# EPFL-VILAB/MultiMAE

Measured on NVIDIA H100. Metric: MultiMAE-B pretrain samples/sec @ bs=128/GPU, higher is better.
Workload: dtype bf16

## Files before the change

### include/multimae_b200.h

```cpp
#ifndef MULTIMAE_B200_H_
#define MULTIMAE_B200_H_

#include <stdint.h>

#ifdef __cplusplus
extern "C" {
#endif

#define MMAE_ABI_VERSION 15

int mmae_abi_version(void);
const char* mmae_last_error(void);
int64_t mmae_launch_count(void);

int mmae_profile_gemm(int enable);
int mmae_profile_gemm_read(double* flops, double* ms, int64_t* launches);
int64_t mmae_profile_gemm_dump(char* buf_host, int64_t capacity);

typedef struct mmae_gemm_epilogue {
  float alpha;
  int act;
  int accumulate;
  int reserved;
  const float* bias;
  const float* residual;
  const void* dgelu_z;
  void* preact_bf16;
  float* out_f32;
  void* out_bf16;
  int64_t ld_residual, ld_dgelu_z, ld_preact, ld_out_f32, ld_out_bf16;
} mmae_gemm_epilogue;

int mmae_gemm_set_variant(int variant);
int mmae_gemm_set_tma_store(int enable);
int mmae_set_pdl(int enable);
int mmae_set_sm_budget(int sms);
int mmae_set_wgrad_stream(int enable);

int mmae_gemm_bf16(const void* A, int64_t lda, int a_mn_major, const void* B, int64_t ldb, int b_mn_major,
                   int M, int N, int K, int split_k, const mmae_gemm_epilogue* ep, void* stream);

int mmae_cast_f32_to_bf16(const float* src, void* dst_bf16, int64_t n, void* stream);
int mmae_cast_colsum_f32(const float* src, int64_t ld_src, void* dst_bf16, int64_t ld_dst, float* colsum,
                         int M, int N, void* stream);
int mmae_colsum_bf16(const void* src_bf16, int64_t ld_src, float* colsum, int M, int N, void* stream);
int mmae_gelu_bf16(const void* z, void* io, int64_t n, int backward, void* stream);
int mmae_dgelu_colsum_bf16(const void* z, void* dz, int64_t ld, float* colsum, int M, int N, void* stream);
int mmae_set_fuse_gelu(int enable);
int mmae_add_bf16_f32(const float* x, const void* y_bf16, float* out, int64_t n, void* stream);
int mmae_transpose_bf16(const void* src, int64_t ld_src, void* dst, int64_t ld_dst, int M, int N, void* stream);

int mmae_layernorm_forward(const float* x, int64_t ldx, const float* gamma, const float* beta, void* y_bf16,
                           int64_t ldy, float* y_f32, int64_t ldyf, float* mean, float* rstd, int M, int D,
// ... 318 lines not shown
```

### multimae_b200/_lib.py

```python
import ctypes
import os

_HERE = os.path.dirname(os.path.abspath(__file__))
LIB_PATH = os.path.join(_HERE, "libmultimae_b200.so")

c_void_p = ctypes.c_void_p
c_int = ctypes.c_int
c_i64 = ctypes.c_int64
c_float = ctypes.c_float


class GemmEpilogue(ctypes.Structure):
    _fields_ = [
        ("alpha", c_float),
        ("act", c_int),
        ("accumulate", c_int),
        ("reserved", c_int),
        ("bias", c_void_p),
        ("residual", c_void_p),
        ("dgelu_z", c_void_p),
        ("preact_bf16", c_void_p),
        ("out_f32", c_void_p),
        ("out_bf16", c_void_p),
        ("ld_residual", c_i64),
        ("ld_dgelu_z", c_i64),
        ("ld_preact", c_i64),
        ("ld_out_f32", c_i64),
        ("ld_out_bf16", c_i64),
    ]


MAX_TASKS = 8
c_float_p = c_void_p
POS_MODES = {"bicubic": 0, "bilinear": 1}


class EmbedLayout(ctypes.Structure):
    _fields_ = [
        ("num_tasks", c_int),
        ("grid_h", c_int * MAX_TASKS), ("grid_w", c_int * MAX_TASKS),
        ("tok_offset", c_int * (MAX_TASKS + 1)),
        ("k_offset", c_int * (MAX_TASKS + 1)),
        ("patch", c_int * MAX_TASKS), ("channels", c_int * MAX_TASKS),
        ("is_semseg", c_int * MAX_TASKS), ("num_classes", c_int * MAX_TASKS),
    ]


class EmbedInputs(ctypes.Structure):
    _fields_ = [("data", c_void_p * MAX_TASKS), ("class_emb", c_void_p * MAX_TASKS)]


# ... 232 lines not shown
    "mmae_block_f32_saved_bytes": (c_i64, [c_int] * 5),
    "mmae_block_f32_workspace_bytes": (c_i64, [c_int] * 5),
    "mmae_block_f32_forward": (c_int, [c_void_p, c_void_p, c_int, c_int, c_int, c_int, c_int, c_float, c_void_p, c_void_p,
                                       ctypes.POINTER(BlockParams), c_void_p, c_void_p, c_void_p]),
    "mmae_block_f32_backward": (c_int, [c_void_p, c_void_p, c_void_p, c_int, c_int, c_int, c_int, c_int, c_void_p, c_void_p,
                                        ctypes.POINTER(BlockParams), ctypes.POINTER(BlockGrads), c_void_p, c_void_p,
                                        c_void_p]),
    "mmae_dechead_f32_saved_bytes": (c_i64, [ctypes.POINTER(DecoderIndex), c_int, c_int, c_int]),
    "mmae_dechead_f32_workspace_bytes": (c_i64, [ctypes.POINTER(DecoderIndex), c_int, c_int, c_int]),
    "mmae_dechead_f32_forward": (c_int, [c_void_p, c_int, ctypes.POINTER(DecoderIndex), c_int, c_int, c_float,
                                         ctypes.POINTER(DecHeadParams), c_void_p, c_void_p, c_void_p, c_void_p]),
    "mmae_dechead_f32_backward": (c_int, [c_void_p, c_int, ctypes.POINTER(DecoderIndex), c_int, c_int,
                                          ctypes.POINTER(DecHeadParams), ctypes.POINTER(DecHeadGrads), c_void_p, c_void_p,
                                          c_void_p, c_void_p, c_void_p]),
    "mmae_dectail_f32_workspace_bytes": (c_i64, [c_int] * 6),
    "mmae_dectail_f32_forward": (c_int, [c_void_p, c_int, c_int, c_int, c_int, c_int, c_int, c_void_p, c_void_p, c_void_p,
                                         c_void_p, c_void_p]),
    "mmae_dectail_f32_backward": (c_int, [c_void_p, c_void_p, c_int, c_int, c_int, c_int, c_int, c_int, c_void_p, c_void_p,
                                          c_void_p, c_void_p, c_void_p, c_void_p]),
    "mmae_standardize_depth_set_variant": (c_int, [c_int]),
    "mmae_standardize_depth": (c_int, [c_void_p, c_void_p, c_int, c_int, c_int, c_int, c_float, c_void_p, c_void_p]),
}

ABI_VERSION = 15


def lib():
    global _lib
    if _lib is not None:
        return _lib
    if not os.path.exists(LIB_PATH):
        raise MmaeError(
            "multimae_b200: %s is missing - build it with `python -m multimae_b200.build` "
            "(there is no CPU fallback)" % LIB_PATH)
    handle = ctypes.CDLL(LIB_PATH)
    for name, (res, args) in SIGNATURES.items():
        fn = getattr(handle, name)
        fn.restype = res
        fn.argtypes = args
    ver = handle.mmae_abi_version()
    if ver != ABI_VERSION:
        raise MmaeError("multimae_b200: ABI version mismatch (library %d, binding %d)" % (ver, ABI_VERSION))
    _lib = handle
    return _lib


def check(rc, what=""):
# ... 13 lines not shown
```

### multimae_b200/csrc/gemm_wgmma.cu

```cuda
#include <algorithm>
#include <cstdlib>

#include "common.cuh"
#include "../../include/multimae_b200.h"

namespace mmae {

void count_launch();
bool gemm_profile_begin(cudaStream_t st, double flops, int M, int N, int K, int flags);
void gemm_profile_end(cudaStream_t st);

namespace {

constexpr int BM = 128;
constexpr int BK = 64;
constexpr int WG_K = 16;
constexpr int GEMM_THREADS = 384;

struct GemmParams {
  int M, N, K;
  int num_kb;
  int kb_per_split;
  int tiles_n;
  int tiles_m;
  int splits;
  int tma_store;
  mmae_gemm_epilogue ep;
};

template <int BN>
struct GemmCfg {
  static constexpr int STAGES = BN == 256 ? 4 : (BN == 192 ? 4 : (BN == 128 ? 6 : 8));
  static constexpr int A_BYTES = BM * BK * 2;
  static constexpr int B_BYTES = BN * BK * 2;
  static constexpr int STAGE_BYTES = A_BYTES + B_BYTES;
  static constexpr int EPI_BOX_BYTES = 64 * 32 * 4;
  static constexpr int EPI_OFFSET = STAGES * STAGE_BYTES;
  static constexpr int BAR_OFFSET = EPI_OFFSET + 2 * 2 * EPI_BOX_BYTES;
  static constexpr int TOTAL = BAR_OFFSET + 256 + 1024;
  static_assert(TOTAL <= 232448, "GEMM exceeds the 227 KB shared-memory limit");
};

struct WorkItem {
  int m0, n0, split, kb_begin, nkb;
};

template <int BN, int CL>
__device__ __forceinline__ WorkItem decode_item(int item, const GemmParams& p, int rank) {
  WorkItem w;
  const int rest = item / p.tiles_n;
  w.n0 = (item - rest * p.tiles_n) * BN;
  w.split = rest / p.tiles_m;
  w.m0 = ((rest - w.split * p.tiles_m) * CL + rank) * BM;
  w.kb_begin = w.split * p.kb_per_split;
  w.nkb = min(p.kb_per_split, p.num_kb - w.kb_begin);
  return w;
}

__device__ __forceinline__ void red_add_v2(float* addr, float a, float b) {
  asm volatile("red.global.add.v2.f32 [%0], {%1, %2};" ::"l"(addr), "f"(a), "f"(b) : "memory");
}

__device__ __forceinline__ void epilogue_pair(float v0, float v1, int row, int n, const GemmParams& p, bool first_split,
                                              bool atomic_out) {
  const mmae_gemm_epilogue& ep = p.ep;
  v0 *= ep.alpha;
  v1 *= ep.alpha;
  if (ep.bias && first_split) {
    const float2 b = __ldg(reinterpret_cast<const float2*>(ep.bias + n));
    v0 += b.x;
    v1 += b.y;
  }
  if (ep.preact_bf16)
    *reinterpret_cast<uint32_t*>(reinterpret_cast<bf16*>(ep.preact_bf16) + int64_t(row) * ep.ld_preact + n) = pack_bf16x2(v0, v1);
  if (ep.act == 1) {
    v0 = gelu_erf(v0);
    v1 = gelu_erf(v1);
  }
  if (ep.dgelu_z) {
    const uint32_t z = __ldg(reinterpret_cast<const unsigned int*>(reinterpret_cast<const bf16*>(ep.dgelu_z) +
                                                                   int64_t(row) * ep.ld_dgelu_z + n));
    const float2 zf = unpack_bf16x2(z);
    v0 *= dgelu_erf(zf.x);
    v1 *= dgelu_erf(zf.y);
  }
  if (ep.residual && first_split) {
    const float2 r = __ldg(reinterpret_cast<const float2*>(ep.residual + int64_t(row) * ep.ld_residual + n));
    v0 += r.x;
    v1 += r.y;
  }
  if (ep.out_f32) {
    float* dst = ep.out_f32 + int64_t(row) * ep.ld_out_f32 + n;
    if (atomic_out) red_add_v2(dst, v0, v1);
    else *reinterpret_cast<float2*>(dst) = make_float2(v0, v1);
  }
  if (ep.out_bf16)
    *reinterpret_cast<uint32_t*>(reinterpret_cast<bf16*>(ep.out_bf16) + int64_t(row) * ep.ld_out_bf16 + n) = pack_bf16x2(v0, v1);
}

template <typename T>
__device__ __forceinline__ void stage_pair(uint8_t* box, int r, int c, float v0, float v1) {
  T* b = reinterpret_cast<T*>(box);
  if constexpr (sizeof(T) == 4) *reinterpret_cast<float2*>(b + r * 32 + c) = make_float2(v0, v1);
  else *reinterpret_cast<uint32_t*>(b + r * 32 + c) = pack_bf16x2(v0, v1);
}

template <int BN, int CL, bool A_MN, bool B_MN>
__global__ void __launch_bounds__(GEMM_THREADS, 1)
    gemm_bf16_kernel(const __grid_constant__ CUtensorMap tmA, const __grid_constant__ CUtensorMap tmB,
                     const __grid_constant__ CUtensorMap tmC, const GemmParams p) {
  pdl_launch_dependents();
  using C = GemmCfg<BN>;
  constexpr int STAGES = C::STAGES;
  constexpr int BH = BN / CL;
  static_assert(!B_MN || BH % 64 == 0, "MN-major B is loaded in 64-column chunks");

  extern __shared__ uint8_t smem_raw[];
  const uint32_t raw_addr = smem_u32(smem_raw);
  uint8_t* smem = smem_raw + ((1024u - (raw_addr & 1023u)) & 1023u);
  uint64_t* full_bar = reinterpret_cast<uint64_t*>(smem + C::BAR_OFFSET);
  uint64_t* empty_bar = full_bar + STAGES;

  const int wg = threadIdx.x >> 7;
  const int rank = CL > 1 ? int(cluster_ctarank()) : 0;
  const int num_items = p.tiles_n * p.tiles_m * p.splits;
  const int first_item = blockIdx.x / CL;
  const int item_stride = gridDim.x / CL;

  if (threadIdx.x == 0) {
    tma_prefetch_desc(&tmA);
    tma_prefetch_desc(&tmB);
    if (p.tma_store) tma_prefetch_desc(&tmC);
#pragma unroll
    for (int s = 0; s < STAGES; ++s) {
      mbar_init(&full_bar[s], 1);
      mbar_init(&empty_bar[s], 2 * CL);
    }
    fence_barrier_init();
  }
  __syncthreads();
  if constexpr (CL > 1) cluster_sync_all();
  pdl_wait();

  if (wg == 0) {
    setmaxnreg_dec<40>();
    if (threadIdx.x == 0) {
      uint32_t it = 0;
      for (int item = first_item; item < num_items; item += item_stride) {
        const WorkItem w = decode_item<BN, CL>(item, p, rank);
        for (int kb = 0; kb < w.nkb; ++kb, ++it) {
          const int s = it % STAGES;
          const uint32_t ph = (it / STAGES) & 1;
          mbar_wait(&empty_bar[s], ph ^ 1u);
          mbar_expect_tx(&full_bar[s], C::STAGE_BYTES);
          uint8_t* sA = smem + s * C::STAGE_BYTES;
          uint8_t* sB = sA + C::A_BYTES;
          const int k0 = (w.kb_begin + kb) * BK;
          if constexpr (!A_MN) {
            tma_load_2d(sA, &tmA, &full_bar[s], k0, w.m0);
          } else {
// ... 9 lines not shown
            }
          } else {
            if constexpr (!B_MN) {
              tma_load_2d_multicast(sB + rank * BH * 128, &tmB, &full_bar[s], k0, w.n0 + rank * BH, 0x3);
            } else {
#pragma unroll
              for (int c = 0; c < BH / 64; ++c)
                tma_load_2d_multicast(sB + (rank * (BH / 64) + c) * (64 * BK * 2), &tmB, &full_bar[s],
                                      w.n0 + rank * BH + c * 64, k0, 0x3);
            }
          }
        }
      }
    }
  } else {
    setmaxnreg_inc<232>();
    const int cw = wg - 1;
    const int t = threadIdx.x & 127;
    const int rl = (t >> 5) * 16 + ((t & 31) >> 2);
    uint8_t* epi = smem + C::EPI_OFFSET + cw * (2 * C::EPI_BOX_BYTES);
    const bool atomic_out = p.ep.accumulate != 0 || p.splits > 1;
    uint32_t it = 0;
    uint32_t boxes = 0;
    auto release = [&](int s) {
      if (t == 0) {
        if constexpr (CL == 1) mbar_arrive(&empty_bar[s]);
        else
          for (int r = 0; r < CL; ++r) mbar_arrive_cluster(mapa_u32(smem_u32(&empty_bar[s]), uint32_t(r)));
      }
    };
    float acc[BN / 2];

    for (int item = first_item; item < num_items; item += item_stride) {
      const WorkItem w = decode_item<BN, CL>(item, p, rank);
      for (int kb = 0; kb < w.nkb; ++kb, ++it) {
        const int s = it % STAGES;
        const uint32_t ph = (it / STAGES) & 1;
        mbar_wait(&full_bar[s], ph);
        const uint32_t a_addr = smem_u32(smem + s * C::STAGE_BYTES) + cw * (64 * BK * 2);
        const uint32_t b_addr = smem_u32(smem + s * C::STAGE_BYTES) + C::A_BYTES;
#pragma unroll
        for (int i = 0; i < BN / 2; ++i) reg_fence(acc[i]);
        wgmma_fence();
#pragma unroll
        for (int j = 0; j < BK / WG_K; ++j) {
          const uint32_t sd = (kb | j) != 0 ? 1u : 0u;
          const uint64_t da = A_MN ? gmma_desc_sw128(a_addr + j * (WG_K * 128), 64 * BK * 2, 1024)
                                   : gmma_desc_sw128(a_addr + j * (WG_K * 2), 16, 1024);
          const uint64_t db = B_MN ? gmma_desc_sw128(b_addr + j * (WG_K * 128), 64 * BK * 2, 1024)
                                   : gmma_desc_sw128(b_addr + j * (WG_K * 2), 16, 1024);
          if constexpr (BN == 256) wgmma_m64n256k16<A_MN ? 1 : 0, B_MN ? 1 : 0>(acc, da, db, sd);
          else if constexpr (BN == 192) wgmma_m64n192k16<A_MN ? 1 : 0, B_MN ? 1 : 0>(acc, da, db, sd);
          else if constexpr (BN == 128) wgmma_m64n128k16<A_MN ? 1 : 0, B_MN ? 1 : 0>(acc, da, db, sd);
          else wgmma_m64n64k16<A_MN ? 1 : 0, B_MN ? 1 : 0>(acc, da, db, sd);
        }
        wgmma_commit();
#pragma unroll
        for (int i = 0; i < BN / 2; ++i) reg_fence(acc[i]);
        wgmma_wait<1>();
        if (kb > 0) release((it - 1) % STAGES);
      }
      wgmma_wait<0>();
#pragma unroll
      for (int i = 0; i < BN / 2; ++i) reg_fence(acc[i]);
      release((it - 1) % STAGES);

      const int row_a = w.m0 + cw * 64 + rl;
      const int row_b = row_a + 8;
      const bool first_split = w.split == 0;
      if (p.tma_store) {
        const float* bias = first_split ? p.ep.bias : nullptr;
        const bool bf16_out = p.tma_store == 1;
#pragma unroll
        for (int b = 0; b < BN / 32; ++b) {
          if (w.n0 + b * 32 >= p.N) break;
          uint8_t* box = bf16_out ? epi + (boxes & 3) * (C::EPI_BOX_BYTES / 2) : epi + (boxes & 1) * C::EPI_BOX_BYTES;
          if (t == 0) {
            if (bf16_out) bulk_wait_read<3>();
            else bulk_wait_read<1>();
          }
          asm volatile("bar.sync %0, 128;" ::"r"(2 + cw) : "memory");
#pragma unroll
          for (int jj = 0; jj < 4; ++jj) {
            const int j = 4 * b + jj;
            const int c = jj * 8 + 2 * (t & 3);
            float v[4] = {acc[4 * j] * p.ep.alpha, acc[4 * j + 1] * p.ep.alpha, acc[4 * j + 2] * p.ep.alpha,
                          acc[4 * j + 3] * p.ep.alpha};
            if (bias && w.n0 + b * 32 + c < p.N) {
              const float2 bb = __ldg(reinterpret_cast<const float2*>(bias + w.n0 + b * 32 + c));
              v[0] += bb.x; v[1] += bb.y; v[2] += bb.x; v[3] += bb.y;
            }
            if (p.ep.act == 1) {
#pragma unroll
              for (int i = 0; i < 4; ++i) v[i] = gelu_erf(v[i]);
            }
            if (bf16_out) {
              stage_pair<bf16>(box, rl, c, v[0], v[1]);
              stage_pair<bf16>(box, rl + 8, c, v[2], v[3]);
            } else {
              stage_pair<float>(box, rl, c, v[0], v[1]);
              stage_pair<float>(box, rl + 8, c, v[2], v[3]);
            }
          }
          fence_proxy_async_smem();
          asm volatile("bar.sync %0, 128;" ::"r"(2 + cw) : "memory");
          if (t == 0) {
            if (p.tma_store == 3) tma_reduce_add_2d(&tmC, box, w.n0 + b * 32, w.m0 + cw * 64);
            else tma_store_2d(&tmC, box, w.n0 + b * 32, w.m0 + cw * 64);
            bulk_commit_group();
          }
          ++boxes;
        }
      } else {
#pragma unroll
        for (int j = 0; j < BN / 8; ++j) {
          if (w.n0 + j * 8 >= p.N) break;
          const int n = w.n0 + j * 8 + 2 * (t & 3);
          if (row_a < p.M) epilogue_pair(acc[4 * j], acc[4 * j + 1], row_a, n, p, first_split, atomic_out);
          if (row_b < p.M) epilogue_pair(acc[4 * j + 2], acc[4 * j + 3], row_b, n, p, first_split, atomic_out);
        }
      }
    }
    if (t == 0 && p.tma_store) bulk_wait_all();
  }
  if constexpr (CL > 1) cluster_sync_all();
}

template <int BN, int CL, bool A_MN, bool B_MN>
int launch_gemm(const CUtensorMap& tmA, const CUtensorMap& tmB, const CUtensorMap& tmC, const GemmParams& p,
                cudaStream_t stream) {
  using C = GemmCfg<BN>;
  auto kern = gemm_bf16_kernel<BN, CL, A_MN, B_MN>;
  cudaLaunchConfig_t cfg;
  memset(&cfg, 0, sizeof(cfg));
  cfg.blockDim = dim3(GEMM_THREADS);
  cfg.dynamicSmemBytes = C::TOTAL;
  cfg.stream = stream;
  cudaLaunchAttribute attr[2];
  attr[0].id = cudaLaunchAttributeClusterDimension;
  attr[0].val.clusterDim.x = CL;
  attr[0].val.clusterDim.y = 1;
  attr[0].val.clusterDim.z = 1;
  attr[1].id = cudaLaunchAttributeProgrammaticStreamSerialization;
  attr[1].val.programmaticStreamSerializationAllowed = 1;
  cfg.attrs = attr;
  cfg.numAttrs = 1;
  static int resident = 0;
  if (resident == 0) {
    MMAE_CUDA_OK(cudaFuncSetAttribute(kern, cudaFuncAttributeMaxDynamicSharedMemorySize, C::TOTAL));
    if constexpr (CL > 1) {
      cfg.gridDim = dim3(CL);
      MMAE_CUDA_OK(cudaOccupancyMaxActiveClusters(&resident, kern, &cfg));
    } else {
      int dev = 0, sms = 0;
      MMAE_CUDA_OK(cudaGetDevice(&dev));
      MMAE_CUDA_OK(cudaDeviceGetAttribute(&sms, cudaDevAttrMultiProcessorCount, dev));
      resident = sms;
    }
    MMAE_CHECK(resident > 0, MMAE_ERR_CUDA, "mmae_gemm_bf16: the GEMM kernel does not fit on an SM");
  }
  const int items = p.tiles_n * p.tiles_m * p.splits;
  const int slots = std::min(resident, std::max(1, sm_count() / CL));
  cfg.gridDim = dim3(std::min(items, slots) * CL);
  const bool prof = gemm_profile_begin(stream, 2.0 * p.M * p.N * p.K, p.M, p.N, p.K,
                                       (A_MN ? 1 : 0) | (B_MN ? 2 : 0) | (p.splits << 8));
  if constexpr (CL == 1) {
    cfg.attrs = attr + 1;
    cfg.numAttrs = pdl_enabled() ? 1 : 0;
  } else {
    cfg.numAttrs = pdl_enabled() ? 2 : 1;
  }
  MMAE_CUDA_OK(cudaLaunchKernelEx(&cfg, kern, tmA, tmB, tmC, p));
  if (prof) gemm_profile_end(stream);
  count_launch();
  MMAE_LAUNCH_OK();
  return MMAE_OK;
}

}
}

using namespace mmae;

static int g_gemm_variant = []() {
  const char* e = getenv("MMAE_GEMM_VARIANT");
  const int v = e ? atoi(e) : -1;
  return v >= -1 && v <= 6 ? v : -1;
}();
static int g_gemm_tma_store = []() {
  const char* e = getenv("MMAE_GEMM_TMA_STORE");
  return e ? (atoi(e) != 0) : 1;
}();

extern "C" int mmae_gemm_set_variant(int variant) {
  MMAE_CHECK(variant >= -1 && variant <= 6, MMAE_ERR_ARG, "mmae_gemm_set_variant: %d (-1 .. 6)", variant);
// ... 1 lines not shown
  return MMAE_OK;
}

extern "C" int mmae_gemm_set_tma_store(int enable) {
  g_gemm_tma_store = enable != 0;
  return MMAE_OK;
}

static int variant_bn(int v) { return v == 0 ? 64 : (v == 1 || v == 6) ? 128 : (v == 3 || v == 5) ? 192 : 256; }

constexpr int KB_PER_ITEM_FIXED = 4;
constexpr int MIN_KB_PER_SPLIT = 16;

extern "C" int mmae_gemm_bf16(const void* A, int64_t lda, int a_mn_major, const void* B, int64_t ldb,
                              int b_mn_major, int M, int N, int K, int split_k, const mmae_gemm_epilogue* ep,
                              void* stream) {
  MMAE_CHECK(A && B && ep, MMAE_ERR_ARG, "mmae_gemm_bf16: null operand");
  MMAE_CHECK(M > 0 && N > 0 && K > 0, MMAE_ERR_ARG, "mmae_gemm_bf16: bad shape M=%d N=%d K=%d", M, N, K);
  MMAE_CHECK(N % 8 == 0, MMAE_ERR_ARG, "mmae_gemm_bf16: N=%d must be a multiple of 8", N);
  MMAE_CHECK(lda % 8 == 0 && ldb % 8 == 0, MMAE_ERR_ARG, "mmae_gemm_bf16: lda/ldb must be multiples of 8");
  MMAE_CHECK((reinterpret_cast<uintptr_t>(A) & 15) == 0 && (reinterpret_cast<uintptr_t>(B) & 15) == 0,
             MMAE_ERR_ARG, "mmae_gemm_bf16: operands must be 16-byte aligned");
  MMAE_CHECK(ep->out_f32 || ep->out_bf16, MMAE_ERR_ARG, "mmae_gemm_bf16: no output");
  const int num_kb = ceil_div(K, BK);
  const int sms = sm_count();
  const int tm = ceil_div(M, BM);
  if (split_k <= 0 && !(ep->out_f32 && !ep->out_bf16 && !ep->preact_bf16 && !ep->dgelu_z && ep->act == 0)) split_k = 1;

  int variant = g_gemm_variant;
  {
    const int cand_var[2] = {1, 2};
    const int nvar = variant >= 0 ? 1 : 2;
    long best_cost = -1;
    int best_split = 1, best_var = variant >= 0 ? variant : 1;
    for (int i = 0; i < nvar; ++i) {
      const int v = variant >= 0 ? variant : cand_var[i];
      const int bn = variant_bn(v), cl = v >= 4 ? 2 : 1;
      if (variant < 0 && bn > 128 && N < bn) continue;
      const long tiles = long(ceil_div(tm, cl)) * ceil_div(N, bn);
      const int slots = std::max(1, sms / cl);
      const int s_lo = split_k > 0 ? split_k : 1;
      const int s_hi = split_k > 0 ? split_k : std::max(1, num_kb / MIN_KB_PER_SPLIT);
      for (int s = s_lo; s <= s_hi; ++s) {
        const int kbps = ceil_div(num_kb, std::min(s, num_kb));
        const long rounds = (tiles * ceil_div(num_kb, kbps) + slots - 1) / slots;
        const long cost = rounds * (bn + 40) * cl * (kbps + KB_PER_ITEM_FIXED);
// ... 30 lines not shown
  int rc;
  if (!a_mn_major) {
    rc = make_tmap_2d_bf16(&tmA, A, (uint64_t)M, (uint64_t)K, (uint64_t)lda, BK, BM);
  } else {
    MMAE_CHECK(M % 8 == 0, MMAE_ERR_ARG, "mmae_gemm_bf16: MN-major A needs M %% 8 == 0");
    rc = make_tmap_2d_bf16(&tmA, A, (uint64_t)K, (uint64_t)M, (uint64_t)lda, 64, BK);
  }
  if (rc) return rc;
  if (!b_mn_major) {
    rc = make_tmap_2d_bf16(&tmB, B, (uint64_t)N, (uint64_t)K, (uint64_t)ldb, BK, BNsel / CLsel);
  } else {
    rc = make_tmap_2d_bf16(&tmB, B, (uint64_t)K, (uint64_t)N, (uint64_t)ldb, 64, BK);
  }
  if (rc) return rc;

  GemmParams p;
  p.M = M; p.N = N; p.K = K;
  p.num_kb = num_kb;
  p.kb_per_split = kb_per_split;
  p.tiles_n = ceil_div(N, BNsel);
  p.tiles_m = ceil_div(tm, CLsel);
  p.splits = split_k;
  p.ep = *ep;
  p.tma_store = 0;
  CUtensorMap tmC = tmA;
  if (g_gemm_tma_store && !ep->preact_bf16 && !ep->dgelu_z && !ep->residual) {
    if (ep->out_bf16 && !ep->out_f32 && split_k == 1 && !ep->accumulate) {
      p.tma_store = 1;
      rc = make_tmap_2d_store(&tmC, ep->out_bf16, 2, (uint64_t)M, (uint64_t)N, (uint64_t)ep->ld_out_bf16);
      if (rc) return rc;
    } else if (ep->out_f32 && !ep->out_bf16 && ep->act == 0) {
      p.tma_store = (split_k > 1 || ep->accumulate) ? 3 : 2;
      rc = make_tmap_2d_store(&tmC, ep->out_f32, 4, (uint64_t)M, (uint64_t)N, (uint64_t)ep->ld_out_f32);
      if (rc) return rc;
    }
  }
  cudaStream_t st = reinterpret_cast<cudaStream_t>(stream);
#define MMAE_DISPATCH(BN_, CL_)                                                                      \
  do {                                                                                               \
    if (!a_mn_major && !b_mn_major) return launch_gemm<BN_, CL_, false, false>(tmA, tmB, tmC, p, st); \
    if (!a_mn_major && b_mn_major) return launch_gemm<BN_, CL_, false, true>(tmA, tmB, tmC, p, st);   \
    if (a_mn_major && !b_mn_major) return launch_gemm<BN_, CL_, true, false>(tmA, tmB, tmC, p, st);   \
    return launch_gemm<BN_, CL_, true, true>(tmA, tmB, tmC, p, st);                                  \
  } while (0)
  if (variant == 4) MMAE_DISPATCH(256, 2);
  if (variant == 6) MMAE_DISPATCH(128, 2);
  if (variant == 5) {
    if (!a_mn_major) return launch_gemm<192, 2, false, false>(tmA, tmB, tmC, p, st);
    return launch_gemm<192, 2, true, false>(tmA, tmB, tmC, p, st);
  }
  if (variant == 0) MMAE_DISPATCH(64, 1);
  if (variant == 3) MMAE_DISPATCH(192, 1);
  if (variant == 2) MMAE_DISPATCH(256, 1);
  MMAE_DISPATCH(128, 1);
#undef MMAE_DISPATCH
}
```

### multimae_b200/csrc/modules.cu

```cuda
#include <cstdlib>

#include "internal.h"

namespace mmae {
namespace {

struct Carver {
  uint8_t* base;
  size_t off = 0;
  explicit Carver(void* b) : base(reinterpret_cast<uint8_t*>(b)) {}
  template <typename T>
  T* take(size_t n) {
    off = align_up(off, 256);
    T* p = reinterpret_cast<T*>(base + off);
    off += n * sizeof(T);
    return p;
  }
};

}


int pick_split(int, int, int) { return 0; }

// ... 17 lines not shown
  ep.bias = b;
  ep.out_bf16 = y;
  ep.ld_out_bf16 = N;
  return mmae_gemm_bf16(x, K, 0, W, K, 0, M, N, K, 1, &ep, st);
}
int linear_f32(const bf16* x, const bf16* W, const float* b, const float* resid, float* y, int M, int N, int K,
               void* st) {
  mmae_gemm_epilogue ep = ep_zero();
  ep.bias = b;
  ep.residual = resid;
  ep.ld_residual = N;
  ep.out_f32 = y;
  ep.ld_out_f32 = N;
  return mmae_gemm_bf16(x, K, 0, W, K, 0, M, N, K, 1, &ep, st);
}
int g_fuse_gelu = []() {
  const char* e = getenv("MMAE_FUSE_GELU");
  return e ? atoi(e) : 0;
}();

int linear_gelu(const bf16* x, const bf16* W, const float* b, bf16* z, bf16* a, int M, int N, int K, void* st) {
  mmae_gemm_epilogue ep = ep_zero();
  ep.bias = b;
  if (g_fuse_gelu) {
    ep.act = 1;
    ep.preact_bf16 = z;
    ep.ld_preact = N;
    ep.out_bf16 = a;
    ep.ld_out_bf16 = N;
    return mmae_gemm_bf16(x, K, 0, W, K, 0, M, N, K, 1, &ep, st);
  }
  ep.out_bf16 = z;
  ep.ld_out_bf16 = N;
  int rc = mmae_gemm_bf16(x, K, 0, W, K, 0, M, N, K, 1, &ep, st);
  if (rc != MMAE_OK) return rc;
  return mmae_gelu_bf16(z, a, int64_t(M) * N, 0, st);
}
int dgrad_bf16(const bf16* dy, int64_t lddy, const bf16* W, const bf16* dgelu_z, bf16* dx, int M, int Nout, int Kin,
               void* st) {
  mmae_gemm_epilogue ep = ep_zero();
  const bool fused = dgelu_z != nullptr && g_fuse_gelu;
  ep.dgelu_z = fused ? dgelu_z : nullptr;
  ep.ld_dgelu_z = Kin;
  ep.out_bf16 = dx;
  ep.ld_out_bf16 = Kin;
  int rc = mmae_gemm_bf16(dy, lddy, 0, W, Kin, 1, M, Kin, Nout, 1, &ep, st);
  if (rc != MMAE_OK || dgelu_z == nullptr || fused) return rc;
  return mmae_gelu_bf16(dgelu_z, dx, int64_t(M) * Kin, 1, st);
}
int dgrad_dgelu_colsum(const bf16* dy, int64_t lddy, const bf16* W, const bf16* z, bf16* dz, float* db, int M, int Nout,
                       int Kin, void* st) {
  if (g_fuse_gelu) {
    int rc = dgrad_bf16(dy, lddy, W, z, dz, M, Nout, Kin, st);
    if (rc != MMAE_OK) return rc;
    return mmae_colsum_bf16(dz, Kin, db, M, Kin, st);
  }
  int rc = dgrad_bf16(dy, lddy, W, nullptr, dz, M, Nout, Kin, st);
  if (rc != MMAE_OK) return rc;
  return mmae_dgelu_colsum_bf16(z, dz, Kin, db, M, Kin, st);
}
int wgrad(const bf16* dy, int64_t lddy, const bf16* x, int64_t ldx, float* dW, int M, int Nout, int Kin, void* st) {
  mmae_gemm_epilogue ep = ep_zero();
  ep.accumulate = 1;
  ep.out_f32 = dW;
  ep.ld_out_f32 = Kin;
  return mmae_gemm_bf16(dy, lddy, 1, x, ldx, 1, Nout, Kin, M, pick_split(Nout, Kin, M), &ep, st);
}

namespace {

#define RUN(expr)             \
  do {                        \
    int _rc = (expr);         \
    if (_rc != MMAE_OK) return _rc; \
  } while (0)

struct BlockSaved {
  bf16 *wqkv, *wproj, *w1, *w2, *h1, *qkv, *o, *h2, *z, *a;
  float *mean1, *rstd1, *mean2, *rstd2, *lse, *x_mid;
  size_t bytes;
};
BlockSaved block_saved(void* base, int B, int N, int D, int H, int hid) {
// ... 721 lines not shown
```

### multimae_b200/kernels.py

```python
import ctypes

import torch

from . import _lib as L


def _need_cuda(*ts):
    for t in ts:
        if t is not None and not t.is_cuda:
            raise L.MmaeError("multimae_b200 kernels need CUDA tensors (no CPU fallback)")


def gemm(A, B, *, a_mn=False, b_mn=False, bias=None, act=0, residual=None, dgelu_z=None, preact=None,
         out_f32=None, out_bf16=None, accumulate=False, split_k=1, alpha=1.0):
    _need_cuda(A, B)
    assert A.dtype == torch.bfloat16 and B.dtype == torch.bfloat16
    assert A.dim() == 2 and B.dim() == 2 and A.stride(1) == 1 and B.stride(1) == 1
    if a_mn:
        K, M = A.shape
    else:
        M, K = A.shape
    if b_mn:
        Kb, N = B.shape
    else:
        N, Kb = B.shape
    assert K == Kb, "contraction mismatch %d vs %d" % (K, Kb)
    ep = L.GemmEpilogue()
    ep.alpha = alpha
    ep.act = act
    ep.accumulate = 1 if accumulate else 0
    for name, ldname, t, dt in (("residual", "ld_residual", residual, torch.float32),
                                ("dgelu_z", "ld_dgelu_z", dgelu_z, torch.bfloat16),
                                ("preact_bf16", "ld_preact", preact, torch.bfloat16),
                                ("out_f32", "ld_out_f32", out_f32, torch.float32),
                                ("out_bf16", "ld_out_bf16", out_bf16, torch.bfloat16)):
        if t is not None:
            assert t.dtype == dt and t.shape[0] == M and t.shape[1] == N and t.stride(1) == 1, name
            setattr(ep, name, t.data_ptr())
            setattr(ep, ldname, t.stride(0))
    if bias is not None:
        assert bias.dtype == torch.float32 and bias.numel() == N
        ep.bias = bias.data_ptr()
    L.check(L.lib().mmae_gemm_bf16(A.data_ptr(), A.stride(0), int(a_mn), B.data_ptr(), B.stride(0), int(b_mn),
                                   M, N, K, split_k, ctypes.byref(ep), L.current_stream()), "mmae_gemm_bf16")


def cast_bf16(src, dst=None):
    _need_cuda(src)
    assert src.dtype == torch.float32 and src.is_contiguous()
    if dst is None:
        dst = torch.empty(src.shape, dtype=torch.bfloat16, device=src.device)
    L.check(L.lib().mmae_cast_f32_to_bf16(src.data_ptr(), dst.data_ptr(), src.numel(), L.current_stream()),
            "mmae_cast_f32_to_bf16")
    return dst


def cast_colsum(src, dst=None, colsum=None):
    _need_cuda(src)
    M, N = src.shape
    L.check(L.lib().mmae_cast_colsum_f32(src.data_ptr(), src.stride(0), L.ptr(dst), dst.stride(0) if dst is not None else 0,
                                         L.ptr(colsum), M, N, L.current_stream()), "mmae_cast_colsum_f32")


def colsum_bf16(src, colsum):
    M, N = src.shape
# ... 79 lines not shown
```

Baseline: 3887.

## Fuse GELU and dGELU+bias-grad column sum into GEMM TMA epilogues

Adds two TMA epilogue modes. One stores both the pre-activation and the GELU output from the forward MLP GEMM. The other loads the saved pre-activation through a TMA ring, applies dGELU to the dgrad result, and reduces per-tile column sums into a bias gradient using a partial buffer and a last-arriver counter. This removes the separate GELU, dGELU and colsum kernels and their extra passes over activation memory in both the fused and unfused settings. In exchange the epilogue grows more complex, with extra barriers, scratch memory and an atomic cross-CTA reduction tail, and the kernel now always takes the extra tensor map argument.

After: 3907, median of 6. Within noise of the previous version (+0.5%).

```diff
diff --git a/include/multimae_b200.h b/include/multimae_b200.h
--- a/include/multimae_b200.h
+++ b/include/multimae_b200.h
@@ -7,7 +7,7 @@
 extern "C" {
 #endif
 
-#define MMAE_ABI_VERSION 15
+#define MMAE_ABI_VERSION 16
 
 int mmae_abi_version(void);
 const char* mmae_last_error(void);
@@ -29,6 +29,9 @@
   float* out_f32;
   void* out_bf16;
   int64_t ld_residual, ld_dgelu_z, ld_preact, ld_out_f32, ld_out_bf16;
+  float* out_colsum;
+  int act_input_bf16;
+  int reserved2;
 } mmae_gemm_epilogue;
 
 int mmae_gemm_set_variant(int variant);
diff --git a/multimae_b200/_lib.py b/multimae_b200/_lib.py
--- a/multimae_b200/_lib.py
+++ b/multimae_b200/_lib.py
@@ -27,6 +27,9 @@
         ("ld_preact", c_i64),
         ("ld_out_f32", c_i64),
         ("ld_out_bf16", c_i64),
+        ("out_colsum", c_void_p),
+        ("act_input_bf16", c_int),
+        ("reserved2", c_int),
     ]
 
 
@@ -305,7 +308,7 @@
     "mmae_standardize_depth": (c_int, [c_void_p, c_void_p, c_int, c_int, c_int, c_int, c_float, c_void_p, c_void_p]),
 }
 
-ABI_VERSION = 15
+ABI_VERSION = 16
 
 
 def lib():
diff --git a/multimae_b200/csrc/gemm_wgmma.cu b/multimae_b200/csrc/gemm_wgmma.cu
--- a/multimae_b200/csrc/gemm_wgmma.cu
+++ b/multimae_b200/csrc/gemm_wgmma.cu
@@ -3,6 +3,7 @@
 
 #include "common.cuh"
 #include "../../include/multimae_b200.h"
+#include "internal.h"
 
 namespace mmae {
 
@@ -16,6 +17,7 @@
 constexpr int BK = 64;
 constexpr int WG_K = 16;
 constexpr int GEMM_THREADS = 384;
+constexpr int Z_RING = 3;
 
 struct GemmParams {
   int M, N, K;
@@ -25,6 +27,8 @@
   int tiles_m;
   int splits;
   int tma_store;
+  float* partial;
+  unsigned int* counters;
   mmae_gemm_epilogue ep;
 };
 
@@ -35,10 +39,12 @@
   static constexpr int B_BYTES = BN * BK * 2;
   static constexpr int STAGE_BYTES = A_BYTES + B_BYTES;
   static constexpr int EPI_BOX_BYTES = 64 * 32 * 4;
+  static constexpr int BF16_BOX_BYTES = 64 * 32 * 2;
   static constexpr int EPI_OFFSET = STAGES * STAGE_BYTES;
   static constexpr int BAR_OFFSET = EPI_OFFSET + 2 * 2 * EPI_BOX_BYTES;
   static constexpr int TOTAL = BAR_OFFSET + 256 + 1024;
   static_assert(TOTAL <= 232448, "GEMM exceeds the 227 KB shared-memory limit");
+  static_assert((2 * STAGES + 8) * 8 + 4 <= 256, "barrier area overflow");
 };
 
 struct WorkItem {
@@ -61,6 +67,8 @@
   asm volatile("red.global.add.v2.f32 [%0], {%1, %2};" ::"l"(addr), "f"(a), "f"(b) : "memory");
 }
 
+__device__ __forceinline__ float bf16_round(float x) { return __bfloat162float(__float2bfloat16_rn(x)); }
+
 __device__ __forceinline__ void epilogue_pair(float v0, float v1, int row, int n, const GemmParams& p, bool first_split,
                                               bool atomic_out) {
   const mmae_gemm_epilogue& ep = p.ep;
@@ -71,18 +79,13 @@
     v0 += b.x;
     v1 += b.y;
   }
-  if (ep.preact_bf16)
-    *reinterpret_cast<uint32_t*>(reinterpret_cast<bf16*>(ep.preact_bf16) + int64_t(row) * ep.ld_preact + n) = pack_bf16x2(v0, v1);
   if (ep.act == 1) {
+    if (ep.act_input_bf16) {
+      v0 = bf16_round(v0);
+      v1 = bf16_round(v1);
+    }
     v0 = gelu_erf(v0);
     v1 = gelu_erf(v1);
-  }
-  if (ep.dgelu_z) {
-    const uint32_t z = __ldg(reinterpret_cast<const unsigned int*>(reinterpret_cast<const bf16*>(ep.dgelu_z) +
-                                                                   int64_t(row) * ep.ld_dgelu_z + n));
-    const float2 zf = unpack_bf16x2(z);
-    v0 *= dgelu_erf(zf.x);
-    v1 *= dgelu_erf(zf.y);
   }
   if (ep.residual && first_split) {
     const float2 r = __ldg(reinterpret_cast<const float2*>(ep.residual + int64_t(row) * ep.ld_residual + n));
@@ -108,7 +111,7 @@
 template <int BN, int CL, bool A_MN, bool B_MN>
 __global__ void __launch_bounds__(GEMM_THREADS, 1)
     gemm_bf16_kernel(const __grid_constant__ CUtensorMap tmA, const __grid_constant__ CUtensorMap tmB,
-                     const __grid_constant__ CUtensorMap tmC, const GemmParams p) {
+                     const __grid_constant__ CUtensorMap tmC, const __grid_constant__ CUtensorMap tmD, const GemmParams p) {
   pdl_launch_dependents();
   using C = GemmCfg<BN>;
   constexpr int STAGES = C::STAGES;
@@ -120,6 +123,8 @@
   uint8_t* smem = smem_raw + ((1024u - (raw_addr & 1023u)) & 1023u);
   uint64_t* full_bar = reinterpret_cast<uint64_t*>(smem + C::BAR_OFFSET);
   uint64_t* empty_bar = full_bar + STAGES;
+  uint64_t* z_bar = empty_bar + STAGES;
+  int* s_flag = reinterpret_cast<int*>(z_bar + 8);
 
   const int wg = threadIdx.x >> 7;
   const int rank = CL > 1 ? int(cluster_ctarank()) : 0;
@@ -131,11 +136,14 @@
     tma_prefetch_desc(&tmA);
     tma_prefetch_desc(&tmB);
     if (p.tma_store) tma_prefetch_desc(&tmC);
+    if (p.tma_store >= 4) tma_prefetch_desc(&tmD);
 #pragma unroll
     for (int s = 0; s < STAGES; ++s) {
       mbar_init(&full_bar[s], 1);
       mbar_init(&empty_bar[s], 2 * CL);
     }
+#pragma unroll
+    for (int s = 0; s < 8; ++s) mbar_init(&z_bar[s], 1);
     fence_barrier_init();
   }
   __syncthreads();
@@ -191,6 +199,8 @@
     const bool atomic_out = p.ep.accumulate != 0 || p.splits > 1;
     uint32_t it = 0;
     uint32_t boxes = 0;
+    uint32_t zph = 0;
+    uint64_t* zb = z_bar + 4 * cw;
     auto release = [&](int s) {
       if (t == 0) {
         if constexpr (CL == 1) mbar_arrive(&empty_bar[s]);
@@ -202,6 +212,7 @@
 
     for (int item = first_item; item < num_items; item += item_stride) {
       const WorkItem w = decode_item<BN, CL>(item, p, rank);
+      const int nbox = min(BN / 32, (p.N - w.n0 + 31) / 32);
       for (int kb = 0; kb < w.nkb; ++kb, ++it) {
         const int s = it % STAGES;
         const uint32_t ph = (it / STAGES) & 1;
@@ -224,6 +235,13 @@
           else wgmma_m64n64k16<A_MN ? 1 : 0, B_MN ? 1 : 0>(acc, da, db, sd);
         }
         wgmma_commit();
+        if (p.tma_store == 5 && kb == 0 && t == 0) {
+          bulk_wait_read<0>();
+          for (int b = 0; b < min(Z_RING, nbox); ++b) {
+            mbar_expect_tx(&zb[b], C::BF16_BOX_BYTES);
+            tma_load_2d(epi + b * C::BF16_BOX_BYTES, &tmD, &zb[b], w.n0 + b * 32, w.m0 + cw * 64);
+          }
+        }
 #pragma unroll
         for (int i = 0; i < BN / 2; ++i) reg_fence(acc[i]);
         wgmma_wait<1>();
@@ -237,18 +255,19 @@
       const int row_a = w.m0 + cw * 64 + rl;
       const int row_b = row_a + 8;
       const bool first_split = w.split == 0;
-      if (p.tma_store) {
-        const float* bias = first_split ? p.ep.bias : nullptr;
-        const bool bf16_out = p.tma_store == 1;
+      if (p.tma_store == 5) {
+        const float* bias = p.ep.bias;
+        const bool colsum = p.ep.out_colsum != nullptr;
+        float csum[BN / 32];
 #pragma unroll
         for (int b = 0; b < BN / 32; ++b) {
-          if (w.n0 + b * 32 >= p.N) break;
-          uint8_t* box = bf16_out ? epi + (boxes & 3) * (C::EPI_BOX_BYTES / 2) : epi + (boxes & 1) * C::EPI_BOX_BYTES;
-          if (t == 0) {
-            if (bf16_out) bulk_wait_read<3>();
-            else bulk_wait_read<1>();
-          }
-          asm volatile("bar.sync %0, 128;" ::"r"(2 + cw) : "memory");
+          csum[b] = 0.f;
+          if (b >= nbox) break;
+          const int slot = b % Z_RING;
+          uint8_t* box = epi + slot * C::BF16_BOX_BYTES;
+          mbar_wait(&zb[slot], (zph >> slot) & 1u);
+          zph ^= 1u << slot;
+          float cs[8];
 #pragma unroll
           for (int jj = 0; jj < 4; ++jj) {
             const int j = 4 * b + jj;
@@ -259,13 +278,106 @@
               const float2 bb = __ldg(reinterpret_cast<const float2*>(bias + w.n0 + b * 32 + c));
               v[0] += bb.x; v[1] += bb.y; v[2] += bb.x; v[3] += bb.y;
             }
-            if (p.ep.act == 1) {
-#pragma unroll
-              for (int i = 0; i < 4; ++i) v[i] = gelu_erf(v[i]);
-            }
-            if (bf16_out) {
+            if (p.ep.act_input_bf16) {
+#pragma unroll
+              for (int i = 0; i < 4; ++i) v[i] = bf16_round(v[i]);
+            }
+            uint32_t* za = reinterpret_cast<uint32_t*>(box) + (rl * 32 + c) / 2;
+            uint32_t* zr = reinterpret_cast<uint32_t*>(box) + ((rl + 8) * 32 + c) / 2;
+            const float2 z0 = unpack_bf16x2(*za), z1 = unpack_bf16x2(*zr);
+            const uint32_t d0 = pack_bf16x2(v[0] * dgelu_erf(z0.x), v[1] * dgelu_erf(z0.y));
+            const uint32_t d1 = pack_bf16x2(v[2] * dgelu_erf(z1.x), v[3] * dgelu_erf(z1.y));
+            *za = d0;
+            *zr = d1;
+            const float2 s0 = row_a < p.M ? unpack_bf16x2(d0) : make_float2(0.f, 0.f);
+            const float2 s1 = row_b < p.M ? unpack_bf16x2(d1) : make_float2(0.f, 0.f);
+            cs[2 * jj] = s0.x + s1.x;
+            cs[2 * jj + 1] = s0.y + s1.y;
+          }
+          fence_proxy_async_smem();
+          asm volatile("bar.sync %0, 128;" ::"r"(2 + cw) : "memory");
+          if (t == 0) {
+            tma_store_2d(&tmC, box, w.n0 + b * 32, w.m0 + cw * 64);
+            bulk_commit_group();
+            if (b >= 1 && b + Z_RING - 1 < nbox) {
+              bulk_wait_read<1>();
+              const int r = (b + Z_RING - 1) % Z_RING;
+              mbar_expect_tx(&zb[r], C::BF16_BOX_BYTES);
+              tma_load_2d(epi + r * C::BF16_BOX_BYTES, &tmD, &zb[r], w.n0 + (b + Z_RING - 1) * 32, w.m0 + cw * 64);
+            }
+          }
+          if (colsum) {
+#pragma unroll
+            for (int h = 0; h < 3; ++h) {
+              const int off = 16 >> h, half = 4 >> h;
+              const bool up = (t & off) != 0;
+#pragma unroll
+              for (int i = 0; i < half; ++i) {
+                const float send = up ? cs[i] : cs[i + half];
+                const float recv = __shfl_xor_sync(0xffffffffu, send, off);
+                cs[i] = (up ? cs[i + half] : cs[i]) + recv;
+              }
+            }
+            csum[b] = cs[0];
+          }
+        }
+        if (colsum) {
+          const int k = ((t >> 4) & 1) * 4 + ((t >> 3) & 1) * 2 + ((t >> 2) & 1);
+          const int lane_col = (k >> 1) * 8 + 2 * (t & 3) + (k & 1);
+          float* red = reinterpret_cast<float*>(epi + Z_RING * C::BF16_BOX_BYTES);
+#pragma unroll
+          for (int b = 0; b < BN / 32; ++b)
+            if (b < nbox) red[(t >> 5) * BN + b * 32 + lane_col] = csum[b];
+          asm volatile("bar.sync 4, 256;" ::: "memory");
+          const float* r0 = reinterpret_cast<const float*>(smem + C::EPI_OFFSET + Z_RING * C::BF16_BOX_BYTES);
+          const float* r1 = r0 + 2 * C::EPI_BOX_BYTES / 4;
+          const int ncol = min(BN, p.N - w.n0);
+          for (int c = cw * 128 + t; c < ncol; c += 256)
+            p.partial[int64_t(w.m0 / BM) * p.N + w.n0 + c] =
+                (((r0[c] + r0[BN + c]) + r0[2 * BN + c]) + r0[3 * BN + c]) +
+                (((r1[c] + r1[BN + c]) + r1[2 * BN + c]) + r1[3 * BN + c]);
+          asm volatile("bar.sync 4, 256;" ::: "memory");
+        }
+      } else if (p.tma_store) {
+        const float* bias = first_split ? p.ep.bias : nullptr;
+        const bool bf16_out = p.tma_store == 1 || p.tma_store == 4;
+        const bool preact = p.tma_store == 4;
+#pragma unroll
+        for (int b = 0; b < BN / 32; ++b) {
+          if (b >= nbox) break;
+          uint8_t* box = preact ? epi + (boxes & 1) * (2 * C::BF16_BOX_BYTES)
+                                : bf16_out ? epi + (boxes & 3) * C::BF16_BOX_BYTES : epi + (boxes & 1) * C::EPI_BOX_BYTES;
+          uint8_t* obox = preact ? box + C::BF16_BOX_BYTES : box;
+          if (t == 0) {
+            if (bf16_out && !preact) bulk_wait_read<3>();
+            else bulk_wait_read<1>();
+          }
+          asm volatile("bar.sync %0, 128;" ::"r"(2 + cw) : "memory");
+#pragma unroll
+          for (int jj = 0; jj < 4; ++jj) {
+            const int j = 4 * b + jj;
+            const int c = jj * 8 + 2 * (t & 3);
+            float v[4] = {acc[4 * j] * p.ep.alpha, acc[4 * j + 1] * p.ep.alpha, acc[4 * j + 2] * p.ep.alpha,
+                          acc[4 * j + 3] * p.ep.alpha};
+            if (bias && w.n0 + b * 32 + c < p.N) {
+              const float2 bb = __ldg(reinterpret_cast<const float2*>(bias + w.n0 + b * 32 + c));
+              v[0] += bb.x; v[1] += bb.y; v[2] += bb.x; v[3] += bb.y;
+            }
+            if (preact) {
               stage_pair<bf16>(box, rl, c, v[0], v[1]);
               stage_pair<bf16>(box, rl + 8, c, v[2], v[3]);
+            }
+            if (p.ep.act == 1) {
+              if (p.ep.act_input_bf16) {
+#pragma unroll
+                for (int i = 0; i < 4; ++i) v[i] = bf16_round(v[i]);
+              }
+#pragma unroll
+              for (int i = 0; i < 4; ++i) v[i] = gelu_erf(v[i]);
+            }
+            if (bf16_out) {
+              stage_pair<bf16>(obox, rl, c, v[0], v[1]);
+              stage_pair<bf16>(obox, rl + 8, c, v[2], v[3]);
             } else {
               stage_pair<float>(box, rl, c, v[0], v[1]);
               stage_pair<float>(box, rl + 8, c, v[2], v[3]);
@@ -275,7 +387,8 @@
           asm volatile("bar.sync %0, 128;" ::"r"(2 + cw) : "memory");
           if (t == 0) {
             if (p.tma_store == 3) tma_reduce_add_2d(&tmC, box, w.n0 + b * 32, w.m0 + cw * 64);
-            else tma_store_2d(&tmC, box, w.n0 + b * 32, w.m0 + cw * 64);
+            else tma_store_2d(&tmC, obox, w.n0 + b * 32, w.m0 + cw * 64);
+            if (preact) tma_store_2d(&tmD, box, w.n0 + b * 32, w.m0 + cw * 64);
             bulk_commit_group();
           }
           ++boxes;
@@ -290,14 +403,60 @@
         }
       }
     }
+    if (p.tma_store == 5 && p.ep.out_colsum != nullptr) {
+      const int Y = p.tiles_m * CL;
+      const int i = cw * 128 + t;
+      int* done = reinterpret_cast<int*>(smem + C::EPI_OFFSET + 2 * C::EPI_BOX_BYTES + Z_RING * C::BF16_BOX_BYTES);
+      float* red = reinterpret_cast<float*>(smem + C::EPI_OFFSET + Z_RING * C::BF16_BOX_BYTES);
+      if (i == 0) *s_flag = 0;
+      __threadfence();
+      asm volatile("bar.sync 4, 256;" ::: "memory");
+      for (int item = first_item + i * item_stride; item < num_items; item += 256 * item_stride) {
+        const int tile_n = item % p.tiles_n;
+        const unsigned int ticket = atomicAdd(&p.counters[tile_n], 1u);
+        if (ticket == unsigned(Y - 1)) {
+          p.counters[tile_n] = 0u;
+          done[atomicAdd(s_flag, 1)] = tile_n;
+        }
+      }
+      asm volatile("bar.sync 4, 256;" ::: "memory");
+      const int ndone = *s_flag;
+      if (ndone > 0) __threadfence();
+      constexpr int GROUPS = BN / 4, G = 256 / GROUPS;
+      const int cg = i % GROUPS, g = i / GROUPS;
+      for (int d = 0; d < ndone; ++d) {
+        const int n0 = done[d] * BN, ncol = min(BN, p.N - n0);
+        float4 a = make_float4(0.f, 0.f, 0.f, 0.f);
+        if (g < G && 4 * cg < ncol) {
+          const float* src = p.partial + n0 + 4 * cg;
+#pragma unroll 8
+          for (int y = g; y < Y; y += G) {
+            const float4 v = __ldcg(reinterpret_cast<const float4*>(src + int64_t(y) * p.N));
+            a.x += v.x; a.y += v.y; a.z += v.z; a.w += v.w;
+          }
+          *reinterpret_cast<float4*>(red + g * BN + 4 * cg) = a;
+        }
+        asm volatile("bar.sync 4, 256;" ::: "memory");
+        if (i < GROUPS && 4 * i < ncol) {
+          float4 tot = *reinterpret_cast<const float4*>(red + 4 * i);
+          for (int gg = 1; gg < G; ++gg) {
+            const float4 v = *reinterpret_cast<const float4*>(red + gg * BN + 4 * i);
+            tot.x += v.x; tot.y += v.y; tot.z += v.z; tot.w += v.w;
+          }
+          float* dst = p.ep.out_colsum + n0 + 4 * i;
+          dst[0] += tot.x; dst[1] += tot.y; dst[2] += tot.z; dst[3] += tot.w;
+        }
+        asm volatile("bar.sync 4, 256;" ::: "memory");
+      }
+    }
     if (t == 0 && p.tma_store) bulk_wait_all();
   }
   if constexpr (CL > 1) cluster_sync_all();
 }
 
 template <int BN, int CL, bool A_MN, bool B_MN>
-int launch_gemm(const CUtensorMap& tmA, const CUtensorMap& tmB, const CUtensorMap& tmC, const GemmParams& p,
-                cudaStream_t stream) {
+int launch_gemm(const CUtensorMap& tmA, const CUtensorMap& tmB, const CUtensorMap& tmC, const CUtensorMap& tmD,
+                const GemmParams& p, cudaStream_t stream) {
   using C = GemmCfg<BN>;
   auto kern = gemm_bf16_kernel<BN, CL, A_MN, B_MN>;
   cudaLaunchConfig_t cfg;
@@ -339,7 +498,7 @@
   } else {
     cfg.numAttrs = pdl_enabled() ? 2 : 1;
   }
-  MMAE_CUDA_OK(cudaLaunchKernelEx(&cfg, kern, tmA, tmB, tmC, p));
+  MMAE_CUDA_OK(cudaLaunchKernelEx(&cfg, kern, tmA, tmB, tmC, tmD, p));
   if (prof) gemm_profile_end(stream);
   count_launch();
   MMAE_LAUNCH_OK();
@@ -387,6 +546,13 @@
   MMAE_CHECK((reinterpret_cast<uintptr_t>(A) & 15) == 0 && (reinterpret_cast<uintptr_t>(B) & 15) == 0,
              MMAE_ERR_ARG, "mmae_gemm_bf16: operands must be 16-byte aligned");
   MMAE_CHECK(ep->out_f32 || ep->out_bf16, MMAE_ERR_ARG, "mmae_gemm_bf16: no output");
+  MMAE_CHECK(ep->act_input_bf16 == 0 || ep->act_input_bf16 == 1, MMAE_ERR_ARG, "mmae_gemm_bf16: act_input_bf16=%d (0 or 1)",
+             ep->act_input_bf16);
+  MMAE_CHECK(!(ep->preact_bf16 || ep->dgelu_z) || (ep->out_bf16 && !ep->out_f32 && !ep->residual), MMAE_ERR_ARG,
+             "mmae_gemm_bf16: preact_bf16 / dgelu_z need out_bf16 and no out_f32 / residual");
+  MMAE_CHECK(!(ep->preact_bf16 && ep->dgelu_z) && !(ep->dgelu_z && ep->act != 0), MMAE_ERR_ARG,
+             "mmae_gemm_bf16: dgelu_z excludes preact_bf16 and act");
+  MMAE_CHECK(!ep->out_colsum || ep->dgelu_z, MMAE_ERR_ARG, "mmae_gemm_bf16: out_colsum needs dgelu_z");
   const int num_kb = ceil_div(K, BK);
   const int sms = sm_count();
   const int tm = ceil_div(M, BM);
@@ -463,9 +629,25 @@
   p.tiles_m = ceil_div(tm, CLsel);
   p.splits = split_k;
   p.ep = *ep;
+  p.partial = nullptr;
+  p.counters = nullptr;
+  cudaStream_t st = reinterpret_cast<cudaStream_t>(stream);
   p.tma_store = 0;
-  CUtensorMap tmC = tmA;
-  if (g_gemm_tma_store && !ep->preact_bf16 && !ep->dgelu_z && !ep->residual) {
+  CUtensorMap tmC = tmA, tmD = tmA;
+  if (ep->preact_bf16 || ep->dgelu_z) {
+    p.tma_store = ep->preact_bf16 ? 4 : 5;
+    rc = make_tmap_2d_store(&tmC, ep->out_bf16, 2, (uint64_t)M, (uint64_t)N, (uint64_t)ep->ld_out_bf16);
+    if (rc) return rc;
+    rc = ep->preact_bf16 ? make_tmap_2d_store(&tmD, ep->preact_bf16, 2, (uint64_t)M, (uint64_t)N, (uint64_t)ep->ld_preact)
+                         : make_tmap_2d_store(&tmD, ep->dgelu_z, 2, (uint64_t)M, (uint64_t)N, (uint64_t)ep->ld_dgelu_z);
+    if (rc) return rc;
+    if (ep->out_colsum) {
+      MMAE_CHECK(p.tiles_n <= int(COLRED_HEADER_FLOATS), MMAE_ERR_ARG, "mmae_gemm_bf16: out_colsum over N=%d is too wide", N);
+      p.partial = colred_scratch(size_t(p.tiles_m) * CLsel * N, st);
+      if (!p.partial) return MMAE_ERR_CUDA;
+      p.counters = colred_counters(p.partial);
+    }
+  } else if (g_gemm_tma_store && !ep->residual) {
     if (ep->out_bf16 && !ep->out_f32 && split_k == 1 && !ep->accumulate) {
       p.tma_store = 1;
       rc = make_tmap_2d_store(&tmC, ep->out_bf16, 2, (uint64_t)M, (uint64_t)N, (uint64_t)ep->ld_out_bf16);
@@ -476,19 +658,18 @@
       if (rc) return rc;
     }
   }
-  cudaStream_t st = reinterpret_cast<cudaStream_t>(stream);
 #define MMAE_DISPATCH(BN_, CL_)                                                                      \
   do {                                                                                               \
-    if (!a_mn_major && !b_mn_major) return launch_gemm<BN_, CL_, false, false>(tmA, tmB, tmC, p, st); \
-    if (!a_mn_major && b_mn_major) return launch_gemm<BN_, CL_, false, true>(tmA, tmB, tmC, p, st);   \
-    if (a_mn_major && !b_mn_major) return launch_gemm<BN_, CL_, true, false>(tmA, tmB, tmC, p, st);   \
-    return launch_gemm<BN_, CL_, true, true>(tmA, tmB, tmC, p, st);                                  \
+    if (!a_mn_major && !b_mn_major) return launch_gemm<BN_, CL_, false, false>(tmA, tmB, tmC, tmD, p, st); \
+    if (!a_mn_major && b_mn_major) return launch_gemm<BN_, CL_, false, true>(tmA, tmB, tmC, tmD, p, st);   \
+    if (a_mn_major && !b_mn_major) return launch_gemm<BN_, CL_, true, false>(tmA, tmB, tmC, tmD, p, st);   \
+    return launch_gemm<BN_, CL_, true, true>(tmA, tmB, tmC, tmD, p, st);                                  \
   } while (0)
   if (variant == 4) MMAE_DISPATCH(256, 2);
   if (variant == 6) MMAE_DISPATCH(128, 2);
   if (variant == 5) {
-    if (!a_mn_major) return launch_gemm<192, 2, false, false>(tmA, tmB, tmC, p, st);
-    return launch_gemm<192, 2, true, false>(tmA, tmB, tmC, p, st);
+    if (!a_mn_major) return launch_gemm<192, 2, false, false>(tmA, tmB, tmC, tmD, p, st);
+    return launch_gemm<192, 2, true, false>(tmA, tmB, tmC, tmD, p, st);
   }
   if (variant == 0) MMAE_DISPATCH(64, 1);
   if (variant == 3) MMAE_DISPATCH(192, 1);
diff --git a/multimae_b200/csrc/modules.cu b/multimae_b200/csrc/modules.cu
--- a/multimae_b200/csrc/modules.cu
+++ b/multimae_b200/csrc/modules.cu
@@ -63,42 +63,32 @@
 int linear_gelu(const bf16* x, const bf16* W, const float* b, bf16* z, bf16* a, int M, int N, int K, void* st) {
   mmae_gemm_epilogue ep = ep_zero();
   ep.bias = b;
-  if (g_fuse_gelu) {
-    ep.act = 1;
-    ep.preact_bf16 = z;
-    ep.ld_preact = N;
-    ep.out_bf16 = a;
-    ep.ld_out_bf16 = N;
-    return mmae_gemm_bf16(x, K, 0, W, K, 0, M, N, K, 1, &ep, st);
-  }
-  ep.out_bf16 = z;
+  ep.act = 1;
+  ep.act_input_bf16 = g_fuse_gelu ? 0 : 1;
+  ep.preact_bf16 = z;
+  ep.ld_preact = N;
+  ep.out_bf16 = a;
   ep.ld_out_bf16 = N;
-  int rc = mmae_gemm_bf16(x, K, 0, W, K, 0, M, N, K, 1, &ep, st);
-  if (rc != MMAE_OK) return rc;
-  return mmae_gelu_bf16(z, a, int64_t(M) * N, 0, st);
+  return mmae_gemm_bf16(x, K, 0, W, K, 0, M, N, K, 1, &ep, st);
+}
+static int dgrad_epilogue(const bf16* dy, int64_t lddy, const bf16* W, const bf16* dgelu_z, float* db, bf16* dx, int M,
+                          int Nout, int Kin, void* st) {
+  mmae_gemm_epilogue ep = ep_zero();
+  ep.dgelu_z = dgelu_z;
+  ep.ld_dgelu_z = Kin;
+  ep.act_input_bf16 = g_fuse_gelu ? 0 : 1;
+  ep.out_colsum = db;
+  ep.out_bf16 = dx;
+  ep.ld_out_bf16 = Kin;
+  return mmae_gemm_bf16(dy, lddy, 0, W, Kin, 1, M, Kin, Nout, 1, &ep, st);
 }
 int dgrad_bf16(const bf16* dy, int64_t lddy, const bf16* W, const bf16* dgelu_z, bf16* dx, int M, int Nout, int Kin,
                void* st) {
-  mmae_gemm_epilogue ep = ep_zero();
-  const bool fused = dgelu_z != nullptr && g_fuse_gelu;
-  ep.dgelu_z = fused ? dgelu_z : nullptr;
-  ep.ld_dgelu_z = Kin;
-  ep.out_bf16 = dx;
-  ep.ld_out_bf16 = Kin;
-  int rc = mmae_gemm_bf16(dy, lddy, 0, W, Kin, 1, M, Kin, Nout, 1, &ep, st);
-  if (rc != MMAE_OK || dgelu_z == nullptr || fused) return rc;
-  return mmae_gelu_bf16(dgelu_z, dx, int64_t(M) * Kin, 1, st);
+  return dgrad_epilogue(dy, lddy, W, dgelu_z, nullptr, dx, M, Nout, Kin, st);
 }
 int dgrad_dgelu_colsum(const bf16* dy, int64_t lddy, const bf16* W, const bf16* z, bf16* dz, float* db, int M, int Nout,
                        int Kin, void* st) {
-  if (g_fuse_gelu) {
-    int rc = dgrad_bf16(dy, lddy, W, z, dz, M, Nout, Kin, st);
-    if (rc != MMAE_OK) return rc;
-    return mmae_colsum_bf16(dz, Kin, db, M, Kin, st);
-  }
-  int rc = dgrad_bf16(dy, lddy, W, nullptr, dz, M, Nout, Kin, st);
-  if (rc != MMAE_OK) return rc;
-  return mmae_dgelu_colsum_bf16(z, dz, Kin, db, M, Kin, st);
+  return dgrad_epilogue(dy, lddy, W, z, db, dz, M, Nout, Kin, st);
 }
 int wgrad(const bf16* dy, int64_t lddy, const bf16* x, int64_t ldx, float* dW, int M, int Nout, int Kin, void* st) {
   mmae_gemm_epilogue ep = ep_zero();
diff --git a/multimae_b200/kernels.py b/multimae_b200/kernels.py
--- a/multimae_b200/kernels.py
+++ b/multimae_b200/kernels.py
@@ -12,8 +12,8 @@
 
 
 def gemm(A, B, *, a_mn=False, b_mn=False, bias=None, act=0, residual=None, dgelu_z=None, preact=None,
-         out_f32=None, out_bf16=None, accumulate=False, split_k=1, alpha=1.0):
-    _need_cuda(A, B)
+         out_f32=None, out_bf16=None, accumulate=False, split_k=1, alpha=1.0, out_colsum=None, act_input_bf16=False):
+    _need_cuda(A, B, out_colsum)
     assert A.dtype == torch.bfloat16 and B.dtype == torch.bfloat16
     assert A.dim() == 2 and B.dim() == 2 and A.stride(1) == 1 and B.stride(1) == 1
     if a_mn:
@@ -29,6 +29,7 @@
     ep.alpha = alpha
     ep.act = act
     ep.accumulate = 1 if accumulate else 0
+    ep.act_input_bf16 = 1 if act_input_bf16 else 0
     for name, ldname, t, dt in (("residual", "ld_residual", residual, torch.float32),
                                 ("dgelu_z", "ld_dgelu_z", dgelu_z, torch.bfloat16),
                                 ("preact_bf16", "ld_preact", preact, torch.bfloat16),
@@ -41,6 +42,9 @@
     if bias is not None:
         assert bias.dtype == torch.float32 and bias.numel() == N
         ep.bias = bias.data_ptr()
+    if out_colsum is not None:
+        assert out_colsum.dtype == torch.float32 and out_colsum.numel() == N and out_colsum.is_contiguous()
+        ep.out_colsum = out_colsum.data_ptr()
     L.check(L.lib().mmae_gemm_bf16(A.data_ptr(), A.stride(0), int(a_mn), B.data_ptr(), B.stride(0), int(b_mn),
                                    M, N, K, split_k, ctypes.byref(ep), L.current_stream()), "mmae_gemm_bf16")
 
```
